# sxontheway/milliEye

Hardware: AMD Instinct MI355X
Metric: frames/sec YOLOv3-416+fusion @batch32, 1/2/4/8 MI355X; mAP@0.5 vs ref (higher is better)
Workload: dtype f32; 1 GPU; yolov3.cfg 416x416 fp32 inference, batch=32 per GPU, full milliEye: Darknet.forward -> NMS -> Network.forward mode 0 (R-CNN head + radar fusion, 2 radar boxes/frame) -> output rows, synthetic frames U[0,1), deterministic trained-like weights; stage=full, batch_per_gpu=32, global_batch=32, img_size=416, parallelism=frames sharded over 1 GPU(s), one process per GPU, no data-path collective, rccl_ranks=0, full=False, output_rows_last_step=6449, rois_last_step=6449

## Files before the change

### include/millieye_hip.h

```cpp
#ifndef MILLIEYE_HIP_H
#define MILLIEYE_HIP_H

#include <stdint.h>

#ifdef __cplusplus
extern "C" {
#endif

#define ME_ABI_VERSION 13

#define ME_E_BADARG (-1)
#define ME_E_NULLPTR (-2)
#define ME_E_ALIGN (-3)
#define ME_E_TOOBIG (-4)

#define ME_ACT_LINEAR 0
#define ME_ACT_LEAKY 1
#define ME_ACT_SIGMOID 2

int me_abi_version(void);
const char* me_last_error(void);
int me_device_query(int32_t* cu_count, int32_t* clock_khz, int32_t* lds_bytes);

typedef struct me_conv_desc {
  const float* x;
  const float* wgt;
  const float* scale;
  const float* shift;
  const float* res;
  float* y;
  int64_t x_pitch;
  int64_t res_pitch;
  int64_t y_pitch;
  int32_t n, h, w, cin;
  int32_t cout, ksize, stride, pad;
  int32_t ho, wo;
  int32_t act;
  int32_t upsample;
  int32_t x_nchw;
  int32_t tile;
  int32_t split_k;
  void* workspace;
  int64_t workspace_bytes;
  const float* wgt_tiled;
  int32_t* tile_counters;
  int64_t tile_counters_len;
  uint32_t tap_mask[4];
  int32_t tap_mask_cols;
  int32_t reserved0;
} me_conv_desc;
int me_conv2d_f32(const me_conv_desc* d, void* stream);
int64_t me_conv2d_workspace_bytes(const me_conv_desc* d);
int64_t me_conv2d_flops(const me_conv_desc* d);

typedef struct me_pool_desc {
  const float* x;
  float* y;
  int64_t x_pitch, y_pitch;
  int32_t n, h, w, c;
  int32_t size, stride, pad, zero_ext;
  int32_t ho, wo;
} me_pool_desc;
int me_maxpool_f32(const me_pool_desc* d, void* stream);

int me_upsample_f32(const float* x, int64_t x_pitch, float* y, int64_t y_pitch, int32_t n, int32_t h,
                    int32_t w, int32_t c, int32_t factor, void* stream);
int me_add_f32(const float* a, int64_t a_pitch, const float* b, int64_t b_pitch, float* y, int64_t y_pitch,
               int64_t pixels, int32_t c, void* stream);
int me_copy_f32(const float* x, int64_t x_pitch, float* y, int64_t y_pitch, int64_t pixels, int32_t c,
                void* stream);
int me_nhwc_to_nchw_f32(const float* x, int64_t x_pitch, float* y, int32_t n, int32_t h, int32_t w, int32_t c,
                        void* stream);

typedef struct me_yolo_desc {
  const float* x;
  float* out;
  int64_t x_pitch;
  int32_t n, g, num_anchors, num_classes;
  int32_t rows_total, row_offset;
  float stride;
  float anchors[16];
} me_yolo_desc;
int me_yolo_decode_f32(const me_yolo_desc* d, void* stream);

typedef struct me_nms_desc {
  float* pred;
// ... 312 lines not shown
```

### millieye_amd/csrc/conv.hip

```cpp
#include <stdlib.h>

#include "common.h"
#include "dma.h"

#include "conv32_common.h"

namespace me32 {
int launch_p8_tile(const ConvP& p, int tile, hipStream_t stream);
bool ws1x1_f32_eligible(const ConvP& p);
int launch_ws1x1_f32(const ConvP& p, hipStream_t stream);
bool ws3x3_f32_eligible(const ConvP& p);
int launch_ws3x3_f32(const ConvP& p, hipStream_t stream);
bool stem_mfma_eligible(const ConvP& p);
int launch_stem_mfma(const ConvP& p, hipStream_t stream);
}

namespace {

template <int BM, int BN, int BK, int WR, int WC, int ABL = 0, int PRIO = 0>
__global__ __launch_bounds__(256) void conv_igemm_f32(ConvP p) {
  static_assert(WR * WC == 4, "4 waves per workgroup");
  constexpr int TM = BM / WR, TN = BN / WC;
  constexpr int MT = TM / 32, NT = TN / 32;
  static_assert(MT >= 1 && NT >= 1, "wave tile must hold at least one 32x32 MFMA tile");
  constexpr int LP = BK + 4;
  constexpr int CH = BK / 4;
  constexpr int A_IT = (BM * CH + 255) / 256;
  constexpr int B_IT = (BN * CH + 255) / 256;

  extern __shared__ __attribute__((aligned(16))) float smem[];
  float* As = smem;
  float* Bs = smem + 2 * BM * LP;

  const int tid = threadIdx.x;
  const int lane = tid & 63;
  const int wave = tid >> 6;
  const int wr = wave / WC, wc = wave % WC;
  const int r32 = lane & 31, hh = lane >> 5;

  int tile_m, tile_n;
  {
    const int nwg = p.tiles_m * p.tiles_n;
    const int bid = blockIdx.x;
    const int q = nwg >> 3, r = nwg & 7;
    const int xcd = bid & 7, idx = bid >> 3;
    const int wg = (xcd < r ? xcd * (q + 1) : r * (q + 1) + (xcd - r) * q) + idx;
    tile_n = wg % p.tiles_n;
// ... 1282 lines not shown
             d->wo, ho, wo);
  ME_REQUIRE((long long)d->n * d->ho * d->wo < (1ll << 31), ME_E_TOOBIG, "me_conv2d_f32: too many output pixels");
  p.x = d->x; p.wgt = d->wgt; p.wgt_tiled = d->wgt_tiled; p.scale = d->scale; p.shift = d->shift; p.res = d->res; p.y = d->y;
  p.x_pitch = d->x_pitch; p.res_pitch = d->res_pitch; p.y_pitch = d->y_pitch;
  p.n = d->n; p.h = d->h; p.w = d->w; p.cin = d->cin; p.cout = d->cout; p.ks = d->ksize;
  p.stride = d->stride; p.pad = d->pad; p.ho = d->ho; p.wo = d->wo; p.act = d->act; p.ups = d->upsample;
  p.x_nchw = d->x_nchw;
  p.M = d->n * d->ho * d->wo;
  p.ktot = d->ksize * d->ksize * d->cin;
  magic_u32((unsigned)(d->ho * d->wo), &p.hw_m, &p.hw_s);
  magic_u32((unsigned)d->wo, &p.wo_m, &p.wo_s);
  p.cs = p.stages = p.tiles_m = p.tiles_n = p.bulk = p.gn = p.kord = 0;
  p.partial = nullptr;
  p.splitk = 1;
  p.sps = 0;
  p.counters = d->tile_counters_len > 0 ? d->tile_counters : nullptr;
  p.counters_len = p.counters ? d->tile_counters_len : 0;
  p.mask_cols = d->tap_mask_cols > 0 ? d->tap_mask_cols : 0;
  for (int i = 0; i < 4; ++i) p.tapmask[i] = d->tap_mask[i];
  return 0;
}

}

extern "C" {

int64_t me_conv2d_flops(const me_conv_desc* d) {
  if (!d) return 0;
  return 2ll * d->n * d->ho * d->wo * (int64_t)d->cout * d->ksize * d->ksize * d->cin;
}

int64_t me_conv2d_workspace_bytes(const me_conv_desc* d) {
  ConvP p;
  if (!d || fill_params(d, p) != 0 || d->cin <= 4) return 0;
  if ((d->tile >= 41 && d->tile <= 45) || d->tile == 47) {
    static const int shape[7][2] = {{128, 128}, {128, 64}, {64, 64}, {128, 32}, {256, 128}, {0, 0}, {64, 64}};
    const int bm = shape[d->tile - 41][0], bn = shape[d->tile - 41][1];
    const long long tiles = (long long)((p.M + bm - 1) / bm) * ((p.cout + bn - 1) / bn);
    const int split = d->split_k > 0 ? d->split_k : 4;
    return (int64_t)(tiles % 256) * split * bm * bn * (int64_t)sizeof(float);
  }
  const ConvPlan plan = plan_conv(p, d->tile, d->split_k > 0 ? d->split_k : kMaxSplit);
  const int split = d->split_k > 0 ? d->split_k : plan.splitk;
  return split > 1 ? (int64_t)split * p.M * p.cout * (int64_t)sizeof(float) : 0;
}

int me_conv2d_f32(const me_conv_desc* d, void* stream_) {
  hipStream_t stream = reinterpret_cast<hipStream_t>(stream_);
  ConvP p;
  int rc = fill_params(d, p);
  if (rc) return rc;
  ME_REQUIRE(d->x && d->wgt && d->scale && d->shift && d->y, ME_E_NULLPTR, "me_conv2d_f32: null tensor pointer");
  ME_REQUIRE(d->upsample == 1 || d->upsample == 2, ME_E_BADARG, "me_conv2d_f32: upsample must be 1 or 2");
  ME_REQUIRE(d->act >= 0 && d->act <= 2, ME_E_BADARG, "me_conv2d_f32: unknown activation %d", d->act);
  ME_REQUIRE(d->y_pitch >= d->cout, ME_E_BADARG, "me_conv2d_f32: y_pitch < cout");

  if (d->cin <= 4) {
    ME_REQUIRE(d->ksize == 3, ME_E_BADARG, "me_conv2d_f32: cin <= 4 needs ksize 3 (direct stem kernel)");
    ME_REQUIRE(d->cout <= SC_MAXCOUT, ME_E_TOOBIG, "me_conv2d_f32: small-cin kernel supports cout <= %d", SC_MAXCOUT);
    ME_REQUIRE(d->res == nullptr && d->upsample == 1, ME_E_BADARG,
               "me_conv2d_f32: small-cin kernel has no residual/upsample epilogue");
    ME_REQUIRE(d->x_nchw || d->x_pitch >= d->cin, ME_E_BADARG, "me_conv2d_f32: x_pitch < cin");
    ME_REQUIRE(me::aligned16(d->y), ME_E_ALIGN, "me_conv2d_f32: y not 16-byte aligned");
    if (d->tile == 0 && me32::stem_mfma_eligible(p)) return me32::launch_stem_mfma(p, stream);
    if (d->cin == 3 && (d->y_pitch & 3) == 0 && d->tile != 91) {
      const unsigned mb = (unsigned)((p.M + 255) / 256);
      if (d->cout % 32 == 0) {
        hipLaunchKernelGGL(conv_stem3_f32<32>, dim3(mb, d->cout / 32), dim3(256), 0, stream, p);
        return me::check_launch("conv_stem3_f32");
      }
      if (d->cout % 16 == 0) {
        hipLaunchKernelGGL(conv_stem3_f32<16>, dim3(mb, d->cout / 16), dim3(256), 0, stream, p);
        return me::check_launch("conv_stem3_f32");
      }
    }
    const long long threads = (long long)p.M * (((p.cout + 7) & ~7) >> 3);
    const unsigned blocks = (unsigned)((threads + 255) / 256);
    if (d->cin == 3)
      hipLaunchKernelGGL(conv_smallcin_f32<3>, dim3(blocks), dim3(256), 0, stream, p);
    else
      hipLaunchKernelGGL(conv_smallcin_f32<4>, dim3(blocks), dim3(256), 0, stream, p);
    return me::check_launch("conv_smallcin_f32");
  }

  ME_REQUIRE(!d->x_nchw, ME_E_BADARG, "me_conv2d_f32: NCHW input only supported for cin <= 4");
  ME_REQUIRE(d->cin % 4 == 0, ME_E_BADARG, "me_conv2d_f32: cin %% 4 != 0 (cin=%d)", d->cin);
  ME_REQUIRE(d->x_pitch >= d->cin && d->x_pitch % 4 == 0, ME_E_ALIGN, "me_conv2d_f32: x_pitch must be >= cin, %% 4");
  ME_REQUIRE(me::aligned16(d->x) && me::aligned16(d->wgt), ME_E_ALIGN, "me_conv2d_f32: x / wgt not 16-byte aligned");
// ... 91 lines not shown
```

### millieye_amd/engine.py

```python
import ctypes as C
import os

import torch

from . import hip

__all__ = ["DarknetEngine", "ConvWeights", "pick_tap_module", "invalidate_weights", "bump_versions"]

_ALIGN = 256

_EPOCH = [0]


def invalidate_weights():
    _EPOCH[0] += 1


def bump_versions(*tensors):
    torch.autograd.graph.increment_version(tensors)

_DTYPES = ("f32", "bf16", "f16")
_TORCH_HALF = {"bf16": torch.bfloat16, "f16": torch.float16}


def _resolve(idx, current):
    idx = int(idx)
    return current + idx if idx < 0 else idx


def pick_tap_module(module_defs):
    if len(module_defs) > 8 and module_defs[8]["type"] == "convolutional":
        return 8
    yolos = [i for i, d in enumerate(module_defs) if d["type"] == "yolo"]
    if len(yolos) < 2:
        return None
    tap = None
    for i in range(yolos[0] + 1, yolos[1]):
        d = module_defs[i]
        if d["type"] == "convolutional" and int(d["filters"]) == 256:
            tap = i
    return tap


class ConvWeights:

    def __init__(self, conv, bn=None, dtype="f32", cin_pad=0, cout_pad=0):
        self.conv, self.bn = conv, bn
        self.dtype, self.cin_pad, self.cout_pad = dtype, cin_pad, cout_pad
        self.wgt = self.scale = self.shift = None
        self.wgt_tiled = None
        self.want_rot = False
        self.rot = self.rot_tiled = None
        self.want_parity, self.parity, self.parity_stamp = False, None, None
        self._stamp = None

    def _sources(self):
        cp = self.conv._parameters
        ts = [cp["weight"]]
        if cp.get("bias") is not None:
            ts.append(cp["bias"])
        if self.bn is not None:
            bp, bb = self.bn._parameters, self.bn._buffers
            ts += [bp["weight"], bp["bias"], bb["running_mean"], bb["running_var"]]
        return ts

    def stamp(self):
        return tuple((t.data_ptr(), t._version) for t in self._sources()) + (_EPOCH[0],)

    def _prepare_packed_f32(self, device):
        conv, bn = self.conv, self.bn
        w = conv.weight
        cout, cin, k, k2 = w.shape
        if k != k2:
            return None
        srcs = [w] + [t for t in ((conv.bias,) if conv.bias is not None else ())]
        if bn is not None:
            srcs += [bn.weight, bn.bias, bn.running_mean, bn.running_var]
        if not all(t.device == device and t.dtype == torch.float32 and t.is_contiguous() for t in srcs):
            return None
        f32 = dict(device=device, dtype=torch.float32)
        realloc = self.wgt is None or self.wgt.device != device or tuple(self.wgt.shape) != (cout, k, k, cin) \
            or self.wgt.dtype != torch.float32
        if realloc:
            self.wgt = torch.empty((cout, k, k, cin), **f32)
            self.scale, self.shift = torch.empty(cout, **f32), torch.empty(cout, **f32)
            self.wgt_tiled = torch.empty((k * k, cin // 16, cout, 16), **f32) if cin % 16 == 0 else None
# ... 2 lines not shown
            self.rot = torch.empty((cin, k, k, cout), **f32)
            self.rot_tiled = torch.empty((k * k, cout // 16, cin, 16), **f32) if cout % 16 == 0 else None
        if realloc:
            self.parity = None
        if self.want_parity and k == 3 and self.parity is None:
            self.parity = torch.empty((4 * cin, 2, 2, cout), **f32)
        return "realloc" if realloc else True

    def _pack_desc(self, d):
        conv, bn = self.conv, self.bn
        ptr = lambda t: t.data_ptr() if t is not None else None
        cout, cin, k, _ = conv.weight.shape
        d.w, d.bias = conv.weight.data_ptr(), ptr(conv.bias)
        d.gamma, d.beta = ptr(bn.weight if bn is not None else None), ptr(bn.bias if bn is not None else None)
        d.mean, d.var = ptr(bn.running_mean if bn is not None else None), ptr(bn.running_var if bn is not None else None)
        d.ohwi, d.tiled = self.wgt.data_ptr(), ptr(self.wgt_tiled)
        d.rot, d.rot_tiled = ptr(self.rot if self.want_rot else None), ptr(self.rot_tiled if self.want_rot else None)
        d.scale, d.shift = self.scale.data_ptr(), self.shift.data_ptr()
        d.parity = ptr(self.parity if self.want_parity else None)
        d.cout, d.cin, d.ksize, d.eps = cout, cin, k, float(bn.eps) if bn is not None else 0.0
        return d

    def _refresh_packed_f32(self, device):
        done = self._prepare_packed_f32(device)
        if done is None:
            return None
        self.parity_stamp = None
        d = self._pack_desc(hip.PackDesc())
        hip.check(hip.lib().me_pack_conv_f32(d.w, d.cout, d.cin, d.ksize, d.bias, d.gamma, d.beta, d.mean, d.var, d.eps, d.ohwi,
                                             d.tiled, d.rot, d.rot_tiled, d.scale, d.shift, hip.stream_ptr()),
                  "me_pack_conv_f32")
        return done

    def refresh(self, device):
        stamp = self.stamp() + (self.want_rot,)
        if stamp == self._stamp and self.wgt is not None and self.wgt.device == device:
            return False
        dev = torch.device(device)
        if self.dtype == "f32" and not self.cin_pad and not self.cout_pad and dev.type == "cuda":
            if dev.index is None:
                dev = torch.device("cuda", torch.cuda.current_device())
            done = self._refresh_packed_f32(dev)
            if done is not None:
                self._stamp = stamp
                return done
        with torch.no_grad():
            w = self.conv.weight.detach().to(device=device, dtype=torch.float32)
            packed = w.permute(0, 2, 3, 1).contiguous()
            cout = w.shape[0]
            if self.bn is not None:
                g = self.bn.weight.detach().to(device, torch.float64)
                b = self.bn.bias.detach().to(device, torch.float64)
                mean = self.bn.running_mean.detach().to(device, torch.float64)
                var = self.bn.running_var.detach().to(device, torch.float64)
                scale = g / torch.sqrt(var + self.bn.eps)
                shift = b - mean * scale
                if self.conv.bias is not None:
                    shift = shift + self.conv.bias.detach().to(device, torch.float64) * scale
            else:
                scale = torch.ones(cout, dtype=torch.float64, device=device)
                if self.conv.bias is not None:
                    shift = self.conv.bias.detach().to(device, torch.float64)
                else:
                    shift = torch.zeros(cout, dtype=torch.float64, device=device)
            scale, shift = scale.to(torch.float32), shift.to(torch.float32)
            cin = packed.shape[3]
            if self.cin_pad > cin:
                packed = torch.nn.functional.pad(packed, (0, self.cin_pad - cin))
            if self.cout_pad > cout:
                extra = self.cout_pad - cout
# ... 418 lines not shown

        lib = hip.lib()
        launches = []
        plan.input_descs = []
        plan.yolo_raw = []
        plan.yolo_descs = []
        plan.conv_descs = []
        flops = 0
        for op in ops:
            kind = op["kind"]
            if kind == "conv":
                x, y = op["x"], op["y"]
                cw = self._conv_weights(op["module"], x.c if x.padded else 0, y.c if y.padded else 0)
                if cw.refresh(device) == "realloc" and self._plans:
                    self._plans.clear()
                dsc = hip.Conv16Desc() if bf16 else hip.ConvDesc()
                if x.external:
                    dsc.x, dsc.x_pitch, dsc.x_nchw = None, x.c, 1
                    plan.input_descs.append(dsc)
                else:
                    dsc.x, dsc.x_pitch = view(x)
                    dsc.x_nchw = 0
                dsc.wgt, dsc.scale, dsc.shift = cw.wgt.data_ptr(), cw.scale.data_ptr(), cw.shift.data_ptr()
                if op["res"] is not None:
                    dsc.res, dsc.res_pitch = view(op["res"])
                else:
                    dsc.res, dsc.res_pitch = None, 0
                dsc.y, dsc.y_pitch = view(y)
                dsc.n, dsc.h, dsc.w, dsc.cin = n, x.h, x.w, x.c
                dsc.cout, dsc.ksize, dsc.stride, dsc.pad = cw.wgt.shape[0], op["k"], op["s"], op["pad"]
                dsc.ho, dsc.wo, dsc.act, dsc.upsample, dsc.tile = op["ho"], op["wo"], op["act"], op["ups"], 0
                dsc.split_k, dsc.workspace, dsc.workspace_bytes = 0, None, 0
                dsc.wgt_tiled = cw.wgt_tiled.data_ptr() if cw.wgt_tiled is not None else None
                if bf16:
                    dsc.y_f32 = 1 if y.esize == 4 else 0
                    dsc.half_type = half_type
                op["launch"] = len(launches)
                op["desc"] = dsc
                launches.append((lib.me_conv2d_h16 if bf16 else lib.me_conv2d_f32, (C.byref(dsc),), dsc,
                                 f"conv{op['module']}"))
                plan.conv_descs.append((op["module"], dsc))
                flops += 2 * n * op["ho"] * op["wo"] * op["cout"] * op["k"] * op["k"] * (x.c - x.padded)
            elif kind == "pool" and bf16:
                x, y = op["x"], op["y"]
                (xp, xpitch), (yp, ypitch) = view(x), view(y)
                launches.append((lib.me_maxpool_h16,
                                 (xp, xpitch, yp, ypitch, n, x.h, x.w, x.c, op["k"], op["s"],
                                  0 if op["zero_ext"] else op["pad"], op["zero_ext"], op["ho"], op["wo"], half_type), None,
                                 f"pool{op['module']}"))
            elif kind == "pool":
                x, y = op["x"], op["y"]
                dsc = hip.PoolDesc()
                dsc.x, dsc.x_pitch = view(x)
                dsc.y, dsc.y_pitch = view(y)
                dsc.n, dsc.h, dsc.w, dsc.c = n, x.h, x.w, x.c
                dsc.size, dsc.stride, dsc.pad, dsc.zero_ext = op["k"], op["s"], (0 if op["zero_ext"] else op["pad"]), \
                    op["zero_ext"]
                dsc.ho, dsc.wo = op["ho"], op["wo"]
                launches.append((lib.me_maxpool_f32, (C.byref(dsc),), dsc, f"pool{op['module']}"))
            elif kind == "upsample":
                x, y = op["x"], op["y"]
                (xp, xpitch), (yp, ypitch) = view(x), view(y)
                launches.append((lib.me_upsample_h16 if x.esize == 2 else lib.me_upsample_f32,
                                 (xp, xpitch, yp, ypitch, n, x.h, x.w, x.c, op["f"]), None,
                                 f"upsample{op['module']}"))
            elif kind == "add":
# ... 250 lines not shown
    _TUNE_FILE_LOADED[0] = True
    try:
        with open(_tune_file()) as fh:
            for k, v in json.load(fh).items():
                _TUNE_CACHE[tuple(int(x) for x in k.split(","))] = (int(v[0]), int(v[1]))
    except (OSError, ValueError):
        pass


def _tune_save():
    import json
    import os
    path = _tune_file()
    try:
        os.makedirs(os.path.dirname(path), exist_ok=True)
        tmp = f"{path}.{os.getpid()}.tmp"
        with open(tmp, "w") as fh:
            json.dump({",".join(str(int(x)) for x in k): list(v) for k, v in _TUNE_CACHE.items()}, fh)
        os.replace(tmp, path)
    except OSError:
        pass


def _autotune(plan, lib):
    import os
    import time

    stream = hip.stream_ptr()
    _tune_load()
    bf16 = plan.dtype in _TORCH_HALF
    conv_fn = lib.me_conv2d_h16 if bf16 else lib.me_conv2d_f32
    todo, keyed = [], []
    for _m, d in plan.conv_descs:
        if d.cin <= 4:
            continue
        key = (d.n, d.h, d.w, d.cin, d.cout, d.ksize, d.stride, d.upsample, int(bool(d.res)))
        if bf16:
            key += (16 + d.y_f32 + 2 * d.half_type,)
        keyed.append((key, d))
        hit = _TUNE_CACHE.get(key)
        if hit is not None:
            d.tile, d.split_k = hit
        else:
            todo.append((key, d))

    def agree_on_rank0():
        import torch.distributed as dist
        if not (dist.is_available() and dist.is_initialized() and dist.get_world_size() > 1):
            return
        if os.environ.get("MILLIEYE_TUNE_SYNC", "0") not in ("1", "true", "on"):
            return
        box = [{k: (int(dd.tile), int(dd.split_k)) for k, dd in keyed} if dist.get_rank() == 0 else None]
        dist.broadcast_object_list(box, src=0)
        _TUNE_STATS["synced"] += 1
        for k, dd in keyed:
            hit0 = box[0].get(k)
            if hit0 is not None:
                dd.tile, dd.split_k = hit0
                _TUNE_CACHE[k] = hit0

    def ensure_workspace(nbytes):
        have = plan.conv_ws.numel() - 256 if plan.conv_ws is not None else 0
        if nbytes > have:
            plan.conv_ws = torch.empty(nbytes + 256, dtype=torch.uint8, device=plan.arena.device)
            have = nbytes
        ptr = plan.conv_ws.data_ptr() + (-plan.conv_ws.data_ptr()) % 256 if plan.conv_ws is not None else None
        for _m2, d2 in plan.conv_descs:
# ... 238 lines not shown
```

### millieye_amd/hip.py

```python
import ctypes as C
import os

import torch

__all__ = ["lib", "available", "default_device", "MeError"]

_HERE = os.path.dirname(os.path.abspath(__file__))
LIB_PATH = os.environ.get("MILLIEYE_HIP_LIB") or os.path.join(_HERE, "libmillieye_hip.so")

ACT_LINEAR, ACT_LEAKY, ACT_SIGMOID = 0, 1, 2


class MeError(RuntimeError):
    pass


class ConvDesc(C.Structure):
    _fields_ = [
        ("x", C.c_void_p), ("wgt", C.c_void_p), ("scale", C.c_void_p), ("shift", C.c_void_p),
        ("res", C.c_void_p), ("y", C.c_void_p),
        ("x_pitch", C.c_int64), ("res_pitch", C.c_int64), ("y_pitch", C.c_int64),
        ("n", C.c_int32), ("h", C.c_int32), ("w", C.c_int32), ("cin", C.c_int32),
        ("cout", C.c_int32), ("ksize", C.c_int32), ("stride", C.c_int32), ("pad", C.c_int32),
        ("ho", C.c_int32), ("wo", C.c_int32),
# ... 108 lines not shown


class AdamDesc(C.Structure):
    _fields_ = [
        ("param", C.c_void_p * ADAM_MAX_TENSORS), ("grad", C.c_void_p * ADAM_MAX_TENSORS),
        ("exp_avg", C.c_void_p * ADAM_MAX_TENSORS), ("exp_avg_sq", C.c_void_p * ADAM_MAX_TENSORS),
        ("numel", C.c_int64 * ADAM_MAX_TENSORS), ("first_chunk", C.c_int32 * ADAM_MAX_TENSORS),
        ("count", C.c_int32), ("decoupled", C.c_int32),
        ("beta2", C.c_float), ("eps", C.c_float), ("weight_decay", C.c_float), ("decay", C.c_float),
        ("one_minus_beta1", C.c_float), ("one_minus_beta2", C.c_float),
        ("neg_step_size", C.c_float), ("bias_correction2_sqrt", C.c_float),
    ]


_STRUCTS = {0: ConvDesc, 1: PoolDesc, 2: YoloDesc, 3: NmsDesc, 4: HeadsDesc, 5: HeadsWeights, 6: Conv16Desc, 7: PackDesc,
            8: Bneck16Desc, 9: AdamDesc}

SIGNATURES = {
    "me_abi_version": (C.c_int, []),
    "me_last_error": (C.c_char_p, []),
    "me_device_query": (C.c_int, [C.POINTER(C.c_int32)] * 3),
    "me_sizeof": (C.c_int32, [C.c_int32]),
    "me_adam_step_f32": (C.c_int, [C.POINTER(AdamDesc), C.c_void_p]),
    "me_adam_chunk": (C.c_int32, []),
    "me_batch_statistics_f32": (C.c_int, [C.c_void_p, C.c_int32, C.c_int32, C.c_void_p, C.c_int32, C.c_int32, C.c_float,
                                          C.c_void_p, C.c_void_p]),
    "me_image_pad_resize_u8_f32": (C.c_int, [C.c_void_p, C.c_int32, C.c_int32, C.c_void_p, C.c_int32, C.c_void_p]),
    "me_image_pad_resize_flip_u8_f32": (C.c_int, [C.c_void_p, C.c_int32, C.c_int32, C.c_void_p, C.c_int32, C.c_int32,
                                                  C.c_void_p]),
    "me_radar_heatmap_f32": (C.c_int, [C.c_void_p, C.c_void_p, C.c_void_p, C.c_int32, C.c_int32, C.c_void_p, C.c_int32,
                                       C.c_void_p]),
    "me_conv2d_f32": (C.c_int, [C.POINTER(ConvDesc), C.c_void_p]),
    "me_conv2d_flops": (C.c_int64, [C.POINTER(ConvDesc)]),
    "me_conv2d_workspace_bytes": (C.c_int64, [C.POINTER(ConvDesc)]),
    "me_compact_sort_rows_f32": (C.c_int, [C.c_void_p, C.c_void_p, C.c_void_p, C.c_int32, C.c_int32, C.c_void_p, C.c_void_p,
                                           C.c_void_p]),
    "me_conv2d_h16": (C.c_int, [C.POINTER(Conv16Desc), C.c_void_p]),
    "me_bneck_h16": (C.c_int, [C.POINTER(Bneck16Desc), C.c_void_p]),
    "me_bneck_h16_supported": (C.c_int, [C.POINTER(Bneck16Desc)]),
    "me_conv2d_h16_workspace_bytes": (C.c_int64, [C.POINTER(Conv16Desc)]),
    "me_maxpool_h16": (C.c_int, [C.c_void_p, C.c_int64, C.c_void_p, C.c_int64] + [C.c_int32] * 11 + [C.c_void_p]),
    "me_upsample_h16": (C.c_int, [C.c_void_p, C.c_int64, C.c_void_p, C.c_int64, C.c_int32, C.c_int32, C.c_int32,
                                   C.c_int32, C.c_int32, C.c_void_p]),
    "me_add_h16": (C.c_int, [C.c_void_p, C.c_int64, C.c_void_p, C.c_int64, C.c_void_p, C.c_int64, C.c_int64,
                             C.c_int32, C.c_int32, C.c_void_p]),
    "me_copy_h16": (C.c_int, [C.c_void_p, C.c_int64, C.c_void_p, C.c_int64, C.c_int64, C.c_int32, C.c_void_p]),
    "me_maxpool_f32": (C.c_int, [C.POINTER(PoolDesc), C.c_void_p]),
    "me_upsample_f32": (C.c_int, [C.c_void_p, C.c_int64, C.c_void_p, C.c_int64, C.c_int32, C.c_int32, C.c_int32,
                                  C.c_int32, C.c_int32, C.c_void_p]),
    "me_add_f32": (C.c_int, [C.c_void_p, C.c_int64, C.c_void_p, C.c_int64, C.c_void_p, C.c_int64, C.c_int64,
                             C.c_int32, C.c_void_p]),
    "me_copy_f32": (C.c_int, [C.c_void_p, C.c_int64, C.c_void_p, C.c_int64, C.c_int64, C.c_int32, C.c_void_p]),
    "me_nhwc_to_nchw_f32": (C.c_int, [C.c_void_p, C.c_int64, C.c_void_p, C.c_int32, C.c_int32, C.c_int32,
                                      C.c_int32, C.c_void_p]),
    "me_yolo_decode_f32": (C.c_int, [C.POINTER(YoloDesc), C.c_void_p]),
    "me_nms_workspace_bytes": (C.c_int64, [C.c_int32, C.c_int32]),
    "me_nms_batched_f32": (C.c_int, [C.POINTER(NmsDesc), C.c_void_p]),
    "me_nms_boxes_f32": (C.c_int, [C.c_void_p, C.c_void_p, C.c_void_p, C.c_int32, C.c_float, C.c_void_p,
                                   C.c_void_p, C.c_void_p, C.c_void_p]),
    "me_gather_class_boxes_f32": (C.c_int, [C.c_void_p, C.c_void_p, C.c_int32, C.c_int32, C.c_int32, C.c_int32,
                                            C.c_int32, C.c_void_p, C.c_void_p, C.c_void_p]),
    "me_roi_heads_f32": (C.c_int, [C.POINTER(HeadsDesc), C.c_void_p]),
    "me_linear_f32": (C.c_int, [C.c_void_p, C.c_int64, C.c_int64, C.c_int32, C.c_void_p, C.c_void_p, C.c_int32, C.c_int32,
                                C.c_void_p, C.c_int64, C.c_void_p]),
    "me_mask_scale_f32": (C.c_int, [C.c_void_p, C.c_void_p, C.c_float, C.c_int64, C.c_void_p, C.c_void_p]),
    "me_dropout_mask_u8": (C.c_int, [C.c_uint64, C.c_float, C.c_int64, C.c_void_p, C.c_void_p]),
# ... 137 lines not shown
        raise MeError(f"{what} failed (rc={rc}): {msg}")


_RAW_STREAM = getattr(torch._C, "_cuda_getCurrentRawStream", None)


def stream_ptr():
    if _RAW_STREAM is not None:
        return C.c_void_p(_RAW_STREAM(torch.cuda.current_device()))
    return C.c_void_p(torch.cuda.current_stream().cuda_stream)


def _require_cuda_f32(t, name):
    if not (isinstance(t, torch.Tensor) and t.is_cuda and t.dtype == torch.float32):
        raise MeError(f"{name} must be a CUDA float32 tensor (got {type(t).__name__}"
                      f"{'' if not isinstance(t, torch.Tensor) else f' {t.device} {t.dtype}'})")


def pack_conv_weight(weight):
    return weight.detach().to(torch.float32).permute(0, 2, 3, 1).contiguous()


def _nhwc_pitch(t, name):
    if t.is_contiguous():
        return t.shape[-1]
    n, h, w, _c = t.shape
    pitch = t.stride(2)
    if t.stride() != (h * w * pitch, w * pitch, pitch, 1):
        raise MeError(f"{name} must be NHWC-contiguous or a channel slice of an NHWC-contiguous tensor")
    return pitch


def conv2d(x_nhwc, wgt_packed, scale, shift, ksize, stride, pad, act, residual=None, upsample=1, out=None,
           x_nchw=False, tile=0, split_k=0, wgt_tiled=None, in_launch_reduce=False, tap_masks=None):
    _require_cuda_f32(x_nhwc, "x")
    if x_nchw:
        n, cin, h, w = x_nhwc.shape
    else:
        n, h, w, cin = x_nhwc.shape
    cout = wgt_packed.shape[0]
    ho = (h + 2 * pad - ksize) // stride + 1
    wo = (w + 2 * pad - ksize) // stride + 1
    if out is None:
        out = torch.empty((n, ho * upsample, wo * upsample, cout), device=x_nhwc.device, dtype=torch.float32)
    d = ConvDesc()
    d.x, d.wgt, d.scale, d.shift = x_nhwc.data_ptr(), wgt_packed.data_ptr(), scale.data_ptr(), shift.data_ptr()
    d.res = residual.data_ptr() if residual is not None else None
    d.y = out.data_ptr()
    d.x_pitch = cin
    if not x_nchw and not x_nhwc.is_contiguous():
        pitch = x_nhwc.stride(2)
        if x_nhwc.stride() != (h * w * pitch, w * pitch, pitch, 1):
            raise MeError("x must be NHWC-contiguous or a channel slice of an NHWC-contiguous tensor")
        d.x_pitch = pitch
    d.res_pitch = _nhwc_pitch(residual, "residual") if residual is not None else 0
    d.y_pitch = _nhwc_pitch(out, "out")
    d.n, d.h, d.w, d.cin, d.cout = n, h, w, cin, cout
    d.ksize, d.stride, d.pad, d.ho, d.wo = ksize, stride, pad, ho, wo
    d.act, d.upsample, d.x_nchw, d.tile, d.split_k = act, upsample, 1 if x_nchw else 0, tile, split_k
    if tile >= 100 and wgt_tiled is None and wgt_packed.shape[3] % 16 == 0:
        wgt_tiled = tile_weights_f32(wgt_packed)
    d.wgt_tiled = wgt_tiled.data_ptr() if wgt_tiled is not None else None
    if tap_masks is not None:
        d.tap_mask_cols = int(tap_masks[0])
        for i, m in enumerate(tap_masks[1]):
            d.tap_mask[i] = int(m)
        d.split_k = 1
    need = lib().me_conv2d_workspace_bytes(C.byref(d)) if tap_masks is None else 0
    keep = None
    if need > 0:
        ws_ptr, keep = _workspace(need, x_nhwc.device, slot="conv")
        d.workspace, d.workspace_bytes = ws_ptr, need
        if in_launch_reduce:
            d.tile_counters, d.tile_counters_len, _keep2 = tile_counters(x_nhwc.device)
    check(lib().me_conv2d_f32(C.byref(d), stream_ptr()), "me_conv2d_f32")
    return out


_CONV_AUTO = {}
_CONV_AUTO_LOADED = [False]


def _conv_auto_file():
    base = os.environ.get("MILLIEYE_TUNE_CACHE")
    if base:
        return base + ".train"
    root = os.environ.get("XDG_CACHE_HOME", os.path.join(os.path.expanduser("~"), ".cache"))
    try:
        gpu = torch.cuda.get_device_name(torch.cuda.current_device()).replace(" ", "_").replace("/", "_")
    except Exception:
        gpu = "unknown"
    return os.path.join(root, "millieye_amd", f"conv_auto_v2_abi{int(lib().me_abi_version())}_{gpu}.json")


# ... 48 lines not shown
                for _ in range(2):
                    scratch = conv2d(x_nhwc, wgt_packed, scale, shift, ksize, stride, pad, act, residual=residual, out=scratch,
                                     tile=tile, split_k=split, wgt_tiled=wgt_tiled, tap_masks=tm)
                a, b = torch.cuda.Event(enable_timing=True), torch.cuda.Event(enable_timing=True)
                a.record()
                for _ in range(3):
                    conv2d(x_nhwc, wgt_packed, scale, shift, ksize, stride, pad, act, residual=residual, out=scratch, tile=tile,
                           split_k=split, wgt_tiled=wgt_tiled, tap_masks=tm)
                b.record()
                torch.cuda.synchronize()
                ms = a.elapsed_time(b) / 3
            except MeError:
                continue
            if ms < best[0]:
                best = (ms, tile, split, masked)
        hit = _CONV_AUTO[key] = (best[1], best[2], best[3])
        _conv_auto_save()
    masked = len(hit) > 2 and hit[2]
    try:
        return conv2d(x_nhwc, wgt_packed, scale, shift, ksize, stride, pad, act, residual=residual, out=out, tile=hit[0],
                      split_k=hit[1], wgt_tiled=wgt_tiled, tap_masks=tap_masks if masked else None)
    except MeError:
        if hit[0] == 0 and not masked:
            raise
        _CONV_AUTO[key] = (0, 0, 0)
        return conv2d(x_nhwc, wgt_packed, scale, shift, ksize, stride, pad, act, residual=residual, out=out, wgt_tiled=wgt_tiled)


def tile_weights_f32(wgt_packed):
    cout, kh, kw, cin = wgt_packed.shape
    if cin % 16:
        raise MeError("tile_weights_f32: cin must be a multiple of 16")
    return wgt_packed.reshape(cout, kh * kw, cin // 16, 16).permute(1, 2, 0, 3).contiguous()


def tile_weights_h16(wgt_packed):
    cout, kh, kw, cin = wgt_packed.shape
    if cin % 32:
        raise MeError("tile_weights_h16: cin must be a multiple of 32")
    return wgt_packed.reshape(cout, kh * kw, cin // 32, 32).permute(1, 2, 0, 3).contiguous()


def conv2d_h16(x, wgt_packed, scale, shift, ksize, stride, pad, act, residual=None, upsample=1, out=None,
                x_nchw=False, y_f32=False, tile=0, split_k=0, half=torch.bfloat16, wgt_tiled=None, debug_ws=None, tap_masks=None):
    if not (isinstance(x, torch.Tensor) and x.is_cuda):
        raise MeError("x must be a CUDA tensor")
    if x_nchw:
        n, cin, h, w = x.shape
    else:
        n, h, w, cin = x.shape
    if cin > 4:
        half = x.dtype
    if half not in HALF_TYPES:
        raise MeError(f"me_conv2d_h16: 16-bit type must be bfloat16 or float16 (got {half})")
    want = torch.float32 if cin <= 4 else half
    if x.dtype != want or wgt_packed.dtype != want:
        raise MeError(f"me_conv2d_h16: x / wgt must be {want} for cin={cin} (got {x.dtype} / {wgt_packed.dtype})")
    cout = wgt_packed.shape[0]
    ho = (h + 2 * pad - ksize) // stride + 1
    wo = (w + 2 * pad - ksize) // stride + 1
    odt = torch.float32 if y_f32 else half
    if out is None:
        out = torch.empty((n, ho * upsample, wo * upsample, cout), device=x.device, dtype=odt)
    if out.dtype != odt or (residual is not None and residual.dtype != odt):
        raise MeError("me_conv2d_h16: out / residual dtype does not match y_f32")
    d = Conv16Desc()
# ... 292 lines not shown
```

Before: 1878 frames/s.

## Add Winograd F(2x2,3x3) MFMA conv path for large 3x3 stride-1 f32 layers

```diff
diff --git a/include/millieye_hip.h b/include/millieye_hip.h
--- a/include/millieye_hip.h
+++ b/include/millieye_hip.h
@@ -52,6 +52,7 @@
 int me_conv2d_f32(const me_conv_desc* d, void* stream);
 int64_t me_conv2d_workspace_bytes(const me_conv_desc* d);
 int64_t me_conv2d_flops(const me_conv_desc* d);
+int me_wino_pack_f32(const float* ohwi, int32_t cout, int32_t cin, float* u, void* stream);
 
 typedef struct me_pool_desc {
   const float* x;
diff --git a/millieye_amd/csrc/conv.hip b/millieye_amd/csrc/conv.hip
--- a/millieye_amd/csrc/conv.hip
+++ b/millieye_amd/csrc/conv.hip
@@ -13,6 +13,7 @@
 int launch_ws3x3_f32(const ConvP& p, hipStream_t stream);
 bool stem_mfma_eligible(const ConvP& p);
 int launch_stem_mfma(const ConvP& p, hipStream_t stream);
+int launch_wino_f32(const ConvP& p, const me_conv_desc* d, hipStream_t stream);
 }
 
 namespace {
@@ -1361,7 +1362,7 @@
 
 int64_t me_conv2d_workspace_bytes(const me_conv_desc* d) {
   ConvP p;
-  if (!d || fill_params(d, p) != 0 || d->cin <= 4) return 0;
+  if (!d || fill_params(d, p) != 0 || d->cin <= 4 || d->tile == 70) return 0;
   if ((d->tile >= 41 && d->tile <= 45) || d->tile == 47) {
     static const int shape[7][2] = {{128, 128}, {128, 64}, {64, 64}, {128, 32}, {256, 128}, {0, 0}, {64, 64}};
     const int bm = shape[d->tile - 41][0], bn = shape[d->tile - 41][1];
@@ -1383,6 +1384,7 @@
   ME_REQUIRE(d->upsample == 1 || d->upsample == 2, ME_E_BADARG, "me_conv2d_f32: upsample must be 1 or 2");
   ME_REQUIRE(d->act >= 0 && d->act <= 2, ME_E_BADARG, "me_conv2d_f32: unknown activation %d", d->act);
   ME_REQUIRE(d->y_pitch >= d->cout, ME_E_BADARG, "me_conv2d_f32: y_pitch < cout");
+  if (d->tile == 70) return me32::launch_wino_f32(p, d, stream);
 
   if (d->cin <= 4) {
     ME_REQUIRE(d->ksize == 3, ME_E_BADARG, "me_conv2d_f32: cin <= 4 needs ksize 3 (direct stem kernel)");
diff --git a/millieye_amd/csrc/conv_wino_f32.hip b/millieye_amd/csrc/conv_wino_f32.hip
--- /dev/null
+++ b/millieye_amd/csrc/conv_wino_f32.hip
@@ -0,0 +1,230 @@
+#include "common.h"
+#include "conv32_common.h"
+
+namespace {
+
+typedef float f4 __attribute__((ext_vector_type(4)));
+
+constexpr int kWT = 64;
+constexpr int kWN = 64;
+constexpr int kCK = 8;
+constexpr int kTS = 16 * kCK + 4;
+constexpr int kAFl = kWT * kTS;
+constexpr int kBFl = 16 * kWN * kCK;
+constexpr int kStageFl = kAFl + kBFl;
+constexpr int kLds = 2 * kStageFl * 4;
+
+struct WinoP {
+  const float* x;
+  const float* u;
+  const float* scale;
+  const float* shift;
+  const float* res;
+  float* y;
+  long long x_pitch, res_pitch, y_pitch;
+  int n, h, w, cin, cout, act;
+  int th, tw, tiles;
+};
+
+__global__ __launch_bounds__(256, 1) void conv_wino_f32(WinoP p) {
+  extern __shared__ __attribute__((aligned(16))) float smem[];
+  const int tid = threadIdx.x, lane = tid & 63, wave = tid >> 6;
+  const int wr = wave & 1, wc = wave >> 1;
+  const int t0 = blockIdx.x * kWT;
+  const int co0 = blockIdx.y * kWN;
+  const int nst = p.cin / kCK;
+  const int thw = p.th * p.tw;
+
+  const int q = tid & 1, px = (tid >> 1) & 15, tl = tid >> 5;
+  const int cu = (tid >> 1) & 63, xb = tid >> 7;
+  int xoff[8];
+#pragma unroll
+  for (int r = 0; r < 8; ++r) {
+    const int tile = t0 + tl + 8 * r;
+    int off = -1;
+    if (tile < p.tiles) {
+      const int nimg = tile / thw, rem = tile - nimg * thw;
+      const int ty = rem / p.tw, tx = rem - ty * p.tw;
+      const int iy = 2 * ty - 1 + (px >> 2), ix = 2 * tx - 1 + (px & 3);
+      if (iy >= 0 && iy < p.h && ix >= 0 && ix < p.w) off = (int)(((long long)(nimg * p.h + iy) * p.w + ix) * p.x_pitch) + 4 * q;
+    }
+    xoff[r] = off;
+  }
+  const float* ubase = p.u + ((long long)(xb * p.cout + co0 + cu) * kCK + 4 * q);
+  const long long ustep_xi = 2ll * p.cout * kCK;
+  const long long ustep_st = 16ll * p.cout * kCK;
+  const int a_dst = tl * kTS + px * kCK + 4 * q;
+  const int b_dst = xb * (kWN * kCK) + cu * kCK + 4 * (q ^ ((cu >> 3) & 1));
+
+  f4 ga[8], gb[8];
+  auto load = [&](int s) {
+#pragma unroll
+    for (int r = 0; r < 8; ++r) {
+      ga[r] = xoff[r] >= 0 ? *reinterpret_cast<const f4*>(p.x + xoff[r] + s * kCK) : f4{0.f, 0.f, 0.f, 0.f};
+      gb[r] = *reinterpret_cast<const f4*>(ubase + s * ustep_st + r * ustep_xi);
+    }
+  };
+  auto store = [&](int buf) {
+    float* as = smem + buf * kStageFl;
+    float* bs = as + kAFl;
+#pragma unroll
+    for (int r = 0; r < 8; ++r) {
+      *reinterpret_cast<f4*>(as + a_dst + r * 8 * kTS) = ga[r];
+      *reinterpret_cast<f4*>(bs + b_dst + r * 2 * kWN * kCK) = gb[r];
+    }
+  };
+
+  f32x16 acc[16];
+#pragma unroll
+  for (int i = 0; i < 16; ++i)
+#pragma unroll
+    for (int e = 0; e < 16; ++e) acc[i][e] = 0.f;
+
+  const int t = lane & 31, hh = lane >> 5;
+  const int a_src = (wr * 32 + t) * kTS + 4 * hh;
+  const int cb = wc * 32 + t;
+  const int b_src = cb * kCK + 4 * (hh ^ ((cb >> 3) & 1));
+
+  load(0);
+  store(0);
+  __syncthreads();
+  for (int s = 0; s < nst; ++s) {
+    const bool more = s + 1 < nst;
+    if (more) load(s + 1);
+    const float* as = smem + (s & 1) * kStageFl;
+    const float* bs = as + kAFl;
+    f4 d[16];
+#pragma unroll
+    for (int i = 0; i < 16; ++i) d[i] = *reinterpret_cast<const f4*>(as + a_src + i * kCK);
+    f4 tt[16];
+#pragma unroll
+    for (int c = 0; c < 4; ++c) {
+      tt[0 + c] = d[0 + c] - d[8 + c];
+      tt[4 + c] = d[4 + c] + d[8 + c];
+      tt[8 + c] = d[8 + c] - d[4 + c];
+      tt[12 + c] = d[4 + c] - d[12 + c];
+    }
+    f4 v[16];
+#pragma unroll
+    for (int r = 0; r < 4; ++r) {
+      v[4 * r + 0] = tt[4 * r + 0] - tt[4 * r + 2];
+      v[4 * r + 1] = tt[4 * r + 1] + tt[4 * r + 2];
+      v[4 * r + 2] = tt[4 * r + 2] - tt[4 * r + 1];
+      v[4 * r + 3] = tt[4 * r + 1] - tt[4 * r + 3];
+    }
+#pragma unroll
+    for (int xi = 0; xi < 16; ++xi) {
+      const f4 b = *reinterpret_cast<const f4*>(bs + xi * (kWN * kCK) + b_src);
+      acc[xi] = __builtin_amdgcn_mfma_f32_32x32x2f32(v[xi].x, b.x, acc[xi], 0, 0, 0);
+      acc[xi] = __builtin_amdgcn_mfma_f32_32x32x2f32(v[xi].y, b.y, acc[xi], 0, 0, 0);
+      acc[xi] = __builtin_amdgcn_mfma_f32_32x32x2f32(v[xi].z, b.z, acc[xi], 0, 0, 0);
+      acc[xi] = __builtin_amdgcn_mfma_f32_32x32x2f32(v[xi].w, b.w, acc[xi], 0, 0, 0);
+    }
+    if (more) store((s + 1) & 1);
+    __syncthreads();
+  }
+
+  const int co = co0 + cb;
+  const float sc = p.scale[co], sh = p.shift[co];
+#pragma unroll
+  for (int e = 0; e < 16; ++e) {
+    const int tile = t0 + wr * 32 + (e & 3) + 8 * (e >> 2) + 4 * hh;
+    if (tile >= p.tiles) continue;
+    const int nimg = tile / thw, rem = tile - nimg * thw;
+    const int ty = rem / p.tw, tx = rem - ty * p.tw;
+    float m[16];
+#pragma unroll
+    for (int i = 0; i < 16; ++i) m[i] = acc[i][e];
+    float a[8];
+#pragma unroll
+    for (int c = 0; c < 4; ++c) {
+      a[c] = m[c] + m[4 + c] + m[8 + c];
+      a[4 + c] = m[4 + c] - m[8 + c] - m[12 + c];
+    }
+    float yv[4];
+#pragma unroll
+    for (int r = 0; r < 2; ++r) {
+      yv[2 * r] = a[4 * r] + a[4 * r + 1] + a[4 * r + 2];
+      yv[2 * r + 1] = a[4 * r + 1] - a[4 * r + 2] - a[4 * r + 3];
+    }
+#pragma unroll
+    for (int k = 0; k < 4; ++k) {
+      const int oy = 2 * ty + (k >> 1), ox = 2 * tx + (k & 1);
+      if (oy >= p.h || ox >= p.w) continue;
+      const long long mm = ((long long)nimg * p.h + oy) * p.w + ox;
+      float val = apply_act(yv[k] * sc + sh, p.act);
+      if (p.res) val += p.res[mm * p.res_pitch + co];
+      p.y[mm * p.y_pitch + co] = val;
+    }
+  }
+}
+
+__global__ __launch_bounds__(256) void wino_pack_f32(const float* __restrict__ ohwi, int cout, int cin, float* __restrict__ u) {
+  const long long i = (long long)blockIdx.x * 256 + threadIdx.x;
+  if (i >= (long long)cout * cin) return;
+  const int co = (int)(i / cin), ci = (int)(i - (long long)co * cin);
+  double g[9];
+#pragma unroll
+  for (int k = 0; k < 9; ++k) g[k] = ohwi[((long long)co * 9 + k) * cin + ci];
+  double gg[12];
+#pragma unroll
+  for (int c = 0; c < 3; ++c) {
+    gg[c] = g[c];
+    gg[3 + c] = 0.5 * (g[c] + g[3 + c] + g[6 + c]);
+    gg[6 + c] = 0.5 * (g[c] - g[3 + c] + g[6 + c]);
+    gg[9 + c] = g[6 + c];
+  }
+  float* dst = u + ((long long)(ci / kCK) * 16 * cout + co) * kCK + ci % kCK;
+#pragma unroll
+  for (int r = 0; r < 4; ++r) {
+    const double a = gg[3 * r], b = gg[3 * r + 1], c = gg[3 * r + 2];
+    const double row[4] = {a, 0.5 * (a + b + c), 0.5 * (a - b + c), c};
+#pragma unroll
+    for (int k = 0; k < 4; ++k) dst[(long long)(4 * r + k) * cout * kCK] = (float)row[k];
+  }
+}
+
+}
+
+namespace me32 {
+
+int launch_wino_f32(const ConvP& c, const me_conv_desc* d, hipStream_t stream) {
+  ME_REQUIRE(d->ksize == 3 && d->stride == 1 && d->pad == 1 && d->upsample == 1 && !d->x_nchw, ME_E_BADARG,
+             "me_conv2d_f32: tile 70 (Winograd F(2x2,3x3)) needs ksize 3, stride 1, pad 1, upsample 1 and NHWC input");
+  ME_REQUIRE(d->tap_mask_cols == 0 && d->split_k <= 1, ME_E_BADARG, "me_conv2d_f32: tile 70 has no tap masks and no K split");
+  ME_REQUIRE(d->cin % kCK == 0 && d->cout % kWN == 0, ME_E_BADARG,
+             "me_conv2d_f32: tile 70 needs cin %% %d == 0 and cout %% %d == 0 (cin=%d cout=%d)", kCK, kWN, d->cin, d->cout);
+  ME_REQUIRE(d->wgt_tiled != nullptr, ME_E_NULLPTR, "me_conv2d_f32: tile 70 reads the Winograd weights (me_wino_pack_f32) from wgt_tiled");
+  ME_REQUIRE(me::aligned16(d->x) && me::aligned16(d->wgt_tiled) && d->x_pitch >= d->cin && d->x_pitch % 4 == 0, ME_E_ALIGN,
+             "me_conv2d_f32: tile 70 needs 16-byte aligned x / weights and x_pitch %% 4 == 0, >= cin");
+  ME_REQUIRE(!d->res || d->res_pitch >= d->cout, ME_E_BADARG, "me_conv2d_f32: res_pitch < cout");
+  ME_REQUIRE((long long)d->n * d->h * d->w * d->x_pitch < (1ll << 31), ME_E_TOOBIG, "me_conv2d_f32: tile 70 input above 2^31 elements");
+  WinoP p;
+  p.x = c.x; p.u = d->wgt_tiled; p.scale = c.scale; p.shift = c.shift; p.res = c.res; p.y = c.y;
+  p.x_pitch = c.x_pitch; p.res_pitch = c.res_pitch; p.y_pitch = c.y_pitch;
+  p.n = c.n; p.h = c.h; p.w = c.w; p.cin = c.cin; p.cout = c.cout; p.act = c.act;
+  p.th = (c.h + 1) / 2; p.tw = (c.w + 1) / 2;
+  const long long tiles = (long long)c.n * p.th * p.tw;
+  ME_REQUIRE(tiles < (1ll << 30), ME_E_TOOBIG, "me_conv2d_f32: tile 70 grid too large");
+  p.tiles = (int)tiles;
+  static bool attr = false;
+  if (!attr) {
+    ME_HIP(hipFuncSetAttribute(reinterpret_cast<const void*>(conv_wino_f32), hipFuncAttributeMaxDynamicSharedMemorySize, kLds));
+    attr = true;
+  }
+  const dim3 grid((unsigned)((tiles + kWT - 1) / kWT), (unsigned)(d->cout / kWN));
+  hipLaunchKernelGGL(conv_wino_f32, grid, dim3(256), kLds, stream, p);
+  return me::check_launch("conv_wino_f32");
+}
+
+}
+
+extern "C" int me_wino_pack_f32(const float* ohwi, int32_t cout, int32_t cin, float* u, void* stream) {
+  ME_REQUIRE(ohwi && u, ME_E_NULLPTR, "me_wino_pack_f32: null pointer");
+  ME_REQUIRE(cout > 0 && cin > 0 && cin % kCK == 0, ME_E_BADARG, "me_wino_pack_f32: needs cin %% %d == 0 (cin=%d)", kCK, cin);
+  const long long n = (long long)cout * cin;
+  ME_REQUIRE((n + 255) / 256 < (1ll << 31), ME_E_TOOBIG, "me_wino_pack_f32: too many filters");
+  hipLaunchKernelGGL(wino_pack_f32, dim3((unsigned)((n + 255) / 256)), dim3(256), 0, reinterpret_cast<hipStream_t>(stream), ohwi,
+                     cout, cin, u);
+  return me::check_launch("wino_pack_f32");
+}
diff --git a/millieye_amd/engine.py b/millieye_amd/engine.py
--- a/millieye_amd/engine.py
+++ b/millieye_amd/engine.py
@@ -18,6 +18,13 @@
 
 def bump_versions(*tensors):
     torch.autograd.graph.increment_version(tensors)
+
+_WINO_MIN_TILES = 4096
+
+
+def _winograd_enabled():
+    return os.environ.get("MILLIEYE_WINOGRAD", "1") not in ("0", "false", "off")
+
 
 _DTYPES = ("f32", "bf16", "f16")
 _TORCH_HALF = {"bf16": torch.bfloat16, "f16": torch.float16}
@@ -52,6 +59,7 @@
         self.want_rot = False
         self.rot = self.rot_tiled = None
         self.want_parity, self.parity, self.parity_stamp = False, None, None
+        self.wgt_wino, self.wino_stamp = None, None
         self._stamp = None
 
     def _sources(self):
@@ -120,10 +128,30 @@
                   "me_pack_conv_f32")
         return done
 
+    def wino_eligible(self):
+        w, conv = self.wgt, self.conv
+        return (_winograd_enabled() and self.dtype == "f32" and not self.cin_pad and not self.cout_pad and w is not None
+                and w.is_cuda and w.dtype == torch.float32 and w.dim() == 4 and w.shape[1:3] == (3, 3) and w.shape[3] % 8 == 0
+                and w.shape[0] % 64 == 0 and tuple(conv.stride) == (1, 1) and tuple(conv.padding) == (1, 1)
+                and tuple(conv.dilation) == (1, 1) and conv.groups == 1)
+
     def refresh(self, device):
         stamp = self.stamp() + (self.want_rot,)
         if stamp == self._stamp and self.wgt is not None and self.wgt.device == device:
-            return False
+            done = False
+        else:
+            done = self._refresh(device, stamp)
+        if self.wino_eligible() and (self.wino_stamp != stamp or self.wgt_wino is None):
+            cout, _, _, cin = self.wgt.shape
+            if self.wgt_wino is None or self.wgt_wino.device != self.wgt.device or self.wgt_wino.shape != (cin // 8, 16, cout, 8):
+                self.wgt_wino = torch.empty((cin // 8, 16, cout, 8), device=self.wgt.device, dtype=torch.float32)
+                done = "realloc"
+            hip.wino_weights_f32(self.wgt, out=self.wgt_wino)
+            self.wino_stamp = stamp
+            done = done or True
+        return done
+
+    def _refresh(self, device, stamp):
         dev = torch.device(device)
         if self.dtype == "f32" and not self.cin_pad and not self.cout_pad and dev.type == "cuda":
             if dev.index is None:
@@ -608,6 +636,9 @@
                 dsc.ho, dsc.wo, dsc.act, dsc.upsample, dsc.tile = op["ho"], op["wo"], op["act"], op["ups"], 0
                 dsc.split_k, dsc.workspace, dsc.workspace_bytes = 0, None, 0
                 dsc.wgt_tiled = cw.wgt_tiled.data_ptr() if cw.wgt_tiled is not None else None
+                if (not bf16 and cw.wgt_wino is not None and not x.external and op["ups"] == 1 and op["k"] == 3 and op["s"] == 1
+                        and op["pad"] == 1 and n * ((op["ho"] + 1) // 2) * ((op["wo"] + 1) // 2) >= _WINO_MIN_TILES):
+                    dsc.tile, dsc.split_k, dsc.wgt_tiled = 70, 1, cw.wgt_wino.data_ptr()
                 if bf16:
                     dsc.y_f32 = 1 if y.esize == 4 else 0
                     dsc.half_type = half_type
@@ -924,7 +955,7 @@
     conv_fn = lib.me_conv2d_h16 if bf16 else lib.me_conv2d_f32
     todo, keyed = [], []
     for _m, d in plan.conv_descs:
-        if d.cin <= 4:
+        if d.cin <= 4 or (not bf16 and d.tile == 70):
             continue
         key = (d.n, d.h, d.w, d.cin, d.cout, d.ksize, d.stride, d.upsample, int(bool(d.res)))
         if bf16:
diff --git a/millieye_amd/hip.py b/millieye_amd/hip.py
--- a/millieye_amd/hip.py
+++ b/millieye_amd/hip.py
@@ -164,6 +164,7 @@
                                        C.c_void_p]),
     "me_conv2d_f32": (C.c_int, [C.POINTER(ConvDesc), C.c_void_p]),
     "me_conv2d_flops": (C.c_int64, [C.POINTER(ConvDesc)]),
+    "me_wino_pack_f32": (C.c_int, [C.c_void_p, C.c_int32, C.c_int32, C.c_void_p, C.c_void_p]),
     "me_conv2d_workspace_bytes": (C.c_int64, [C.POINTER(ConvDesc)]),
     "me_compact_sort_rows_f32": (C.c_int, [C.c_void_p, C.c_void_p, C.c_void_p, C.c_int32, C.c_int32, C.c_void_p, C.c_void_p,
                                            C.c_void_p]),
@@ -367,7 +368,7 @@
 
 
 def conv2d(x_nhwc, wgt_packed, scale, shift, ksize, stride, pad, act, residual=None, upsample=1, out=None,
-           x_nchw=False, tile=0, split_k=0, wgt_tiled=None, in_launch_reduce=False, tap_masks=None):
+           x_nchw=False, tile=0, split_k=0, wgt_tiled=None, in_launch_reduce=False, tap_masks=None, wgt_wino=None):
     _require_cuda_f32(x_nhwc, "x")
     if x_nchw:
         n, cin, h, w = x_nhwc.shape
@@ -395,6 +396,8 @@
     d.act, d.upsample, d.x_nchw, d.tile, d.split_k = act, upsample, 1 if x_nchw else 0, tile, split_k
     if tile >= 100 and wgt_tiled is None and wgt_packed.shape[3] % 16 == 0:
         wgt_tiled = tile_weights_f32(wgt_packed)
+    if tile == 70:
+        wgt_tiled = wgt_wino if wgt_wino is not None else wino_weights_f32(wgt_packed)
     d.wgt_tiled = wgt_tiled.data_ptr() if wgt_tiled is not None else None
     if tap_masks is not None:
         d.tap_mask_cols = int(tap_masks[0])
@@ -509,6 +512,17 @@
     if cin % 16:
         raise MeError("tile_weights_f32: cin must be a multiple of 16")
     return wgt_packed.reshape(cout, kh * kw, cin // 16, 16).permute(1, 2, 0, 3).contiguous()
+
+
+def wino_weights_f32(wgt_packed, out=None):
+    cout, kh, kw, cin = wgt_packed.shape
+    _require_cuda_f32(wgt_packed, "wgt_packed")
+    if (kh, kw) != (3, 3) or cin % 8 or not wgt_packed.is_contiguous():
+        raise MeError("wino_weights_f32: needs contiguous 3x3 OHWI weights with cin % 8 == 0")
+    if out is None:
+        out = torch.empty((cin // 8, 16, cout, 8), device=wgt_packed.device, dtype=torch.float32)
+    check(lib().me_wino_pack_f32(wgt_packed.data_ptr(), cout, cin, out.data_ptr(), stream_ptr()), "me_wino_pack_f32")
+    return out
 
 
 def tile_weights_h16(wgt_packed):
```

After: 1563 frames/s (median of 2 runs). -16.8%, worse.
